# jianfch/stable-ts

Measured on AMD Instinct MI355X. Metric: real-time factor (audio-sec/wall-sec) large-v3 word_timestamps=True, higher is better.
Workload: dtype f16; 1 GPU; large-v3 (random-init, weight recipe BENCH_WEIGHTS = the parity-pinned recipe of tests/test_gpu_f16_depth.py), 10 min synthetic 16 kHz audio per GPU, word_timestamps=True, beam_size=5, 112 decode steps/window, window-parallel batch 20, default regrouping inside the timed pass; mode=transcribe, windows_per_gpu=20, segments=125, words=1670, parallelism=dp1 (windows sharded, no data-path collective)

## Files before the change

stable_ts_amd/csrc/swx_decode.hip:

```cpp
#include "swx_common.h"
#include "swx_kernels.h"
#include "swx_decode.h"

namespace {

constexpr int SEL_T = 1024;
constexpr float NEG_INF = -__builtin_inff();

struct ArgMax { float v; int i; };

__device__ __forceinline__ ArgMax argmax_combine(ArgMax a, ArgMax b)
{
    if (b.v > a.v || (b.v == a.v && b.i < a.i)) return b;
    return a;
}

static_assert(SEL_T == 1024, "block reductions: 16 wave slots");

__device__ ArgMax block_argmax(ArgMax x, ArgMax *sh)
{
    const int wave = threadIdx.x >> 6, lane = threadIdx.x & 63;
#define SWX_ARGMAX_STEP(O) { ArgMax y; y.v = lane_xor<O>(x.v, lane); y.i = lane_xor<O>(x.i, lane); x = argmax_combine(x, y); }
    SWX_ARGMAX_STEP(32) SWX_ARGMAX_STEP(16) SWX_ARGMAX_STEP(8) SWX_ARGMAX_STEP(4) SWX_ARGMAX_STEP(2) SWX_ARGMAX_STEP(1)
    __syncthreads();
    if (lane == 0) sh[wave] = x;
    __syncthreads();
#ifdef SWX_SELECT_R5_REDUCE
    ArgMax r = sh[0];
    for (int w = 1; w < (int)(blockDim.x >> 6); ++w) r = argmax_combine(r, sh[w]);
    return r;
#else
    x = sh[lane & 15];
    SWX_ARGMAX_STEP(8) SWX_ARGMAX_STEP(4) SWX_ARGMAX_STEP(2) SWX_ARGMAX_STEP(1)
    return x;
#endif
#undef SWX_ARGMAX_STEP
}

__device__ float block_max(float x, float *sh)
{
    x = wave_max(x);
    const int wave = threadIdx.x >> 6, lane = threadIdx.x & 63;
    __syncthreads();
    if (lane == 0) sh[wave] = x;
    __syncthreads();
#if defined(SWX_SELECT_R5_REDUCE) || defined(SWX_SELECT_MAX_WALK)
    float r = sh[0];
    for (int w = 1; w < (int)(blockDim.x >> 6); ++w) r = fmaxf(r, sh[w]);
    return r;
#else
    const f32x4 *s4 = (const f32x4 *)sh;
    float r = -__builtin_inff();
#pragma unroll
    for (int q = 0; q < 4; ++q) { const f32x4 v = s4[q]; r = fmaxf(r, fmaxf(fmaxf(v[0], v[1]), fmaxf(v[2], v[3]))); }
    return r;
#endif
}

__device__ float block_sum(float x, float *sh)
{
    x = wave_sum(x);
    const int wave = threadIdx.x >> 6, lane = threadIdx.x & 63;
    __syncthreads();
    if (lane == 0) sh[wave] = x;
    __syncthreads();
    float r = 0.f;
#if defined(SWX_SELECT_R5_REDUCE) || defined(SWX_SELECT_SUM_WALK)
    for (int w = 0; w < (int)(blockDim.x >> 6); ++w) r += sh[w];
#else
    const f32x4 *s4 = (const f32x4 *)sh;
#pragma unroll
    for (int q = 0; q < 4; ++q) { const f32x4 v = s4[q]; r += v[0]; r += v[1]; r += v[2]; r += v[3]; }
#endif
    return r;
}

__device__ __forceinline__ unsigned hash32(unsigned x)
{
    x ^= x >> 16; x *= 0x7feb352du; x ^= x >> 15; x *= 0x846ca68bu; x ^= x >> 16;
    return x;
}

__device__ __forceinline__ float gumbel(uint64_t seed, unsigned row_uid, unsigned step, unsigned idx)
{
    unsigned h = hash32((unsigned)seed ^ hash32(idx + 0x9e3779b9u * (step + 1u)));
    h = hash32(h ^ hash32(row_uid * 0x85ebca6bu + (unsigned)(seed >> 32)));
    const float u = ((float)(h >> 8) + 0.5f) * (1.0f / 16777216.0f);
    return -logf(-logf(u));
}

__device__ __forceinline__ int win_begin(const DecodeBufs &b, int w) { return b.begin ? b.begin[w] : b.n_init; }

__global__ void decode_init_kernel(DecodeBufs b, const int32_t *__restrict__ init_tokens)
{
    const int r = blockIdx.x;
    const int w = r / b.G;
    const int n0 = win_begin(b, w);
    int32_t *row0 = b.tokens[0] + (size_t)r * b.TS;
    int32_t *row1 = b.tokens[1] + (size_t)r * b.TS;
    for (int i = threadIdx.x; i < b.TS; i += blockDim.x) {
        const int32_t t = (i < n0) ? init_tokens[(size_t)w * b.n_init + i] : b.cfg.eot;
        row0[i] = t;
        row1[i] = t;
    }
    if (threadIdx.x == 0) {
        b.pos0[r] = 0;
        b.sum_lp[r] = 0.f;
        b.row_done[r] = 0;
        if (r % b.G == 0) { b.win_done[w] = 0; b.fin_count[w] = 0; }
        if (r == 0) { *b.n_done = 0; *b.step_dev = 0; }
    }
}

__global__ void decode_after_prefill_kernel(DecodeBufs b)
{
    const int r = blockIdx.x;
    const int w = r / b.G;
    const int n0 = win_begin(b, w);
    if (b.anc[0]) {
        for (int p = threadIdx.x; p < b.n_ctx; p += blockDim.x) {
            const int v = (p < n0) ? w * b.G : r;
            b.anc[0][(size_t)r * b.n_ctx + p] = v;
            b.anc[1][(size_t)r * b.n_ctx + p] = v;
        }
    }
    if (threadIdx.x == 0) b.pos0[r] = n0 - 1;
}

__global__ __launch_bounds__(SEL_T) void decode_prefill_logits_kernel(DecodeBufs b, const float *__restrict__ lg2,
                                                                      float *__restrict__ nospeech)
{
    __shared__ __attribute__((aligned(16))) float sh[SEL_T / 64];
    const int r = blockIdx.x, w = r / b.G, V = b.V;
    const float *last = lg2 + ((size_t)w * 2 + 1) * V;
    float *dst = b.logits + (size_t)r * V;
    for (int i = threadIdx.x; i < V; i += SEL_T) dst[i] = last[i];
    if (r % b.G == 0 && nospeech) {
        const float *sot = lg2 + ((size_t)w * 2) * V;
        float mx = NEG_INF;
        for (int i = threadIdx.x; i < V; i += SEL_T) mx = fmaxf(mx, sot[i]);
        mx = block_max(mx, sh);
        float sum = 0.f;
        for (int i = threadIdx.x; i < V; i += SEL_T) sum += expf(sot[i] - mx);
        sum = block_sum(sum, sh);
        if (threadIdx.x == 0) nospeech[w] = (b.cfg.no_speech >= 0) ? expf(sot[b.cfg.no_speech] - mx) / sum : NAN;
    }
}

__global__ __launch_bounds__(SEL_T) void decode_select_kernel(DecodeBufs b, int cur)
{
    const int step = *b.step_dev;
    __shared__ __attribute__((aligned(16))) float shf[SEL_T / 64];
    __shared__ __attribute__((aligned(16))) ArgMax sha[SEL_T / 64];
    __shared__ int sh_last_ts;
    const int r = blockIdx.x, w = r / b.G, V = b.V, tid = threadIdx.x;
    const swx_decode_cfg &c = b.cfg;
    if (b.win_done[w]) return;
    float *lg = b.logits + (size_t)r * V;
    int32_t *tok = b.tokens[cur] + (size_t)r * b.TS;
    const int n0 = win_begin(b, w);
    const int len = n0 + step;
    const int nsamp = step;
    const int tsb = c.timestamp_begin;

    if (c.suppress_blank && nsamp == 0 && tid == 0) { if (c.blank_token >= 0) lg[c.blank_token] = NEG_INF; lg[c.eot] = NEG_INF; }
    for (int i = tid; i < c.n_suppress; i += SEL_T) { const int t = b.suppress[i]; if ((unsigned)t < (unsigned)V) lg[t] = NEG_INF; }
    if (c.min_tokens > 0 && nsamp < c.min_tokens && tid == 0) lg[c.eot] = NEG_INF;
    __syncthreads();

    if (c.apply_timestamp_rules) {
        if (tid == 0) { sh_last_ts = -1; if (c.no_timestamps >= 0) lg[c.no_timestamps] = NEG_INF; }
        __syncthreads();
        int my = -1;
        for (int i = n0 + tid; i < len; i += SEL_T) if (tok[i] >= tsb) my = i;
        if (my >= 0) atomicMax(&sh_last_ts, my);
        __syncthreads();
        const int last_ts_pos = sh_last_ts;
        const bool last_was_ts = nsamp >= 1 && tok[len - 1] >= tsb;
        const bool penult_was_ts = nsamp < 2 || tok[len - 2] >= tsb;
        int lo0 = 0, hi0 = 0;
        if (last_was_ts) { if (penult_was_ts) { lo0 = tsb; hi0 = V; } else { lo0 = 0; hi0 = c.eot; } }
        int hi1 = tsb;
        if (last_ts_pos >= 0) {
            const int tl = tok[last_ts_pos];
            hi1 = (last_was_ts && !penult_was_ts) ? tl : tl + 1;
        }
        int hi2 = 0;
        int lo3 = V;
        if (nsamp == 0) { hi2 = tsb; if (c.max_initial_timestamp_index >= 0) lo3 = tsb + c.max_initial_timestamp_index + 1; }
        float mx_text = NEG_INF, mx_ts = NEG_INF;
        for (int i = tid; i < V; i += SEL_T) {
            float v = lg[i];
            if ((i >= lo0 && i < hi0) || (i >= tsb && i < hi1) || (i < hi2) || (i >= lo3)) { v = NEG_INF; lg[i] = v; }
            if (i < tsb) mx_text = fmaxf(mx_text, v != v ? -NEG_INF : v); else mx_ts = fmaxf(mx_ts, v);
        }
        mx_text = block_max(mx_text, shf);
        mx_ts = block_max(mx_ts, shf);
        float s_ts = 0.f;
        if (mx_ts > NEG_INF)
            for (int i = tsb + tid; i < V; i += SEL_T) s_ts += expf(lg[i] - mx_ts);
        s_ts = block_sum(s_ts, shf);
        const float lse_ts = (mx_ts > NEG_INF) ? mx_ts + logf(s_ts) : NEG_INF;
        if (lse_ts > mx_text)
            for (int i = tid; i < tsb; i += SEL_T) lg[i] = NEG_INF;
        __syncthreads();
    }

    const uint8_t *tmask = b.ts_mask ? b.ts_mask + (size_t)w * 1501 : nullptr;
    float mx = NEG_INF;
    for (int i = tid; i < V; i += SEL_T) {
        float v = lg[i];
        if (tmask && i >= tsb && i - tsb < 1501 && tmask[i - tsb]) v = NEG_INF;
        if (v != v) v = NEG_INF;
        else if (v == NEG_INF) v = -3.4028234663852886e38f;
        else if (v == -NEG_INF) v = 3.4028234663852886e38f;
        lg[i] = v;
        mx = fmaxf(mx, v);
    }
    mx = block_max(mx, shf);
    float se = 0.f;
    for (int i = tid; i < V; i += SEL_T) se += expf(lg[i] - mx);
    se = block_sum(se, shf);
    const float lse = logf(se);

    if (!c.beam) {
        ArgMax best; best.v = NEG_INF; best.i = 0x7fffffff;
        if (c.temperature == 0.f) {
            for (int i = tid; i < V; i += SEL_T) { ArgMax x; x.v = lg[i]; x.i = i; best = argmax_combine(best, x); }
        } else {
            const float invT = 1.0f / c.temperature;
            const unsigned row_uid = b.win_uid ? (unsigned)b.win_uid[r / b.G] * 0x9E3779B1u + (unsigned)(r % b.G) : (unsigned)r;
            const float *qn = c.noise ? c.noise + ((size_t)step * b.M + r) * V : nullptr;
            for (int i = tid; i < V; i += SEL_T) {
                ArgMax x; x.v = lg[i] * invT + (qn ? -logf(qn[i]) : gumbel(c.seed, row_uid, (unsigned)step, (unsigned)i)); x.i = i;
                best = argmax_combine(best, x);
            }
        }
        best = block_argmax(best, sha);
        if (tid == 0) {
            int next = best.i;
            const bool prev_eot = tok[len - 1] == c.eot;
            const float lp = (lg[next] - mx) - lse;
            if (!prev_eot) b.sum_lp[r] += lp; else next = c.eot;
            tok[len] = next;
            if (len < b.n_ctx) b.pos0[r] = len;
            b.row_done[r] = (next == c.eot) ? 1 : 0;
        }
    } else {
        const int K = b.G + 1;
        for (int k = 0; k < K; ++k) {
            ArgMax best; best.v = NEG_INF; best.i = 0x7fffffff;
            for (int i = tid; i < V; i += SEL_T) { ArgMax x; x.v = lg[i]; x.i = i; best = argmax_combine(best, x); }
            best = block_argmax(best, sha);
            if (tid == 0) {
                b.cand_lp[(size_t)r * K + k] = (best.v - mx) - lse;
                b.cand_tok[(size_t)r * K + k] = best.i;
                lg[best.i] = NEG_INF;
            }
            __syncthreads();
        }
    }
}

template <int NV>
__global__ __launch_bounds__(SEL_T) void decode_select_reg_kernel(DecodeBufs b, int cur)
{
    const int step = *b.step_dev;
    __shared__ __attribute__((aligned(16))) float shf[SEL_T / 64];
    __shared__ __attribute__((aligned(16))) ArgMax sha[SEL_T / 64];
    __shared__ float sh_rot[SEL_T];
    __shared__ int sh_last_ts;
    __shared__ float sh_raw;
    const int r = blockIdx.x, w = r / b.G, V = b.V, tid = threadIdx.x;
    const swx_decode_cfg &c = b.cfg;
    if (b.win_done[w]) return;
    float *lg = b.logits + (size_t)r * V;
    int32_t *tok = b.tokens[cur] + (size_t)r * b.TS;
    const int n0 = win_begin(b, w);
    const int len = n0 + step;
    const int nsamp = step;
    const int tsb = c.timestamp_begin;

    if (c.suppress_blank && nsamp == 0 && tid == 0) { if (c.blank_token >= 0) lg[c.blank_token] = NEG_INF; lg[c.eot] = NEG_INF; }
    for (int i = tid; i < c.n_suppress; i += SEL_T) { const int t = b.suppress[i]; if ((unsigned)t < (unsigned)V) lg[t] = NEG_INF; }
    if (c.min_tokens > 0 && nsamp < c.min_tokens && tid == 0) lg[c.eot] = NEG_INF;
    if (c.apply_timestamp_rules && tid == 0) { sh_last_ts = -1; if (c.no_timestamps >= 0) lg[c.no_timestamps] = NEG_INF; }
    __syncthreads();

    float v[NV];
#pragma unroll
    for (int k = 0; k < NV; ++k) { const int i = tid + k * SEL_T; v[k] = i < V ? lg[i] : NEG_INF; }

    if (c.apply_timestamp_rules) {
        int my = -1;
        for (int i = n0 + tid; i < len; i += SEL_T) if (tok[i] >= tsb) my = i;
        if (my >= 0) atomicMax(&sh_last_ts, my);
        __syncthreads();
        const int last_ts_pos = sh_last_ts;
        const bool last_was_ts = nsamp >= 1 && tok[len - 1] >= tsb;
        const bool penult_was_ts = nsamp < 2 || tok[len - 2] >= tsb;
        int lo0 = 0, hi0 = 0;
        if (last_was_ts) { if (penult_was_ts) { lo0 = tsb; hi0 = V; } else { lo0 = 0; hi0 = c.eot; } }
        int hi1 = tsb;
        if (last_ts_pos >= 0) {
            const int tl = tok[last_ts_pos];
            hi1 = (last_was_ts && !penult_was_ts) ? tl : tl + 1;
        }
        int hi2 = 0, lo3 = V;
        if (nsamp == 0) { hi2 = tsb; if (c.max_initial_timestamp_index >= 0) lo3 = tsb + c.max_initial_timestamp_index + 1; }
        float mx_text = NEG_INF, mx_ts = NEG_INF;
#pragma unroll
        for (int k = 0; k < NV; ++k) {
            const int i = tid + k * SEL_T;
            if (i < V) {
                if ((i >= lo0 && i < hi0) || (i >= tsb && i < hi1) || (i < hi2) || (i >= lo3)) v[k] = NEG_INF;
                if (i < tsb) mx_text = fmaxf(mx_text, v[k] != v[k] ? -NEG_INF : v[k]); else mx_ts = fmaxf(mx_ts, v[k]);
            }
        }
        mx_text = block_max(mx_text, shf);
        mx_ts = block_max(mx_ts, shf);
        float s_own = 0.f;
        if (mx_ts > NEG_INF) {
#pragma unroll
            for (int k = 0; k < NV; ++k) { const int i = tid + k * SEL_T; if (i >= tsb && i < V) s_own += expf(v[k] - mx_ts); }
        }
        sh_rot[(tid - tsb) & (SEL_T - 1)] = s_own;
        __syncthreads();
        float s_ts = block_sum(sh_rot[tid], shf);
        const float lse_ts = (mx_ts > NEG_INF) ? mx_ts + logf(s_ts) : NEG_INF;
        if (lse_ts > mx_text) {
#pragma unroll
            for (int k = 0; k < NV; ++k) if (tid + k * SEL_T < tsb) v[k] = NEG_INF;
        }
    }

    const uint8_t *tmask = b.ts_mask ? b.ts_mask + (size_t)w * 1501 : nullptr;
    float mx = NEG_INF;
#pragma unroll
    for (int k = 0; k < NV; ++k) {
        const int i = tid + k * SEL_T;
        if (i < V) {
            float x = v[k];
            if (tmask && i >= tsb && i - tsb < 1501 && tmask[i - tsb]) x = NEG_INF;
            if (x != x) x = NEG_INF;
            else if (x == NEG_INF) x = -3.4028234663852886e38f;
            else if (x == -NEG_INF) x = 3.4028234663852886e38f;
            v[k] = x;
            mx = fmaxf(mx, x);
        }
    }
    mx = block_max(mx, shf);
    float se = 0.f;
#pragma unroll
    for (int k = 0; k < NV; ++k) if (tid + k * SEL_T < V) se += expf(v[k] - mx);
    se = block_sum(se, shf);
    const float lse = logf(se);

    if (!c.beam) {
        ArgMax best; best.v = NEG_INF; best.i = 0x7fffffff;
        float raw_own = 0.f;
        if (c.temperature == 0.f) {
#pragma unroll
            for (int k = 0; k < NV; ++k) {
                const int i = tid + k * SEL_T;
                if (i < V) { ArgMax x; x.v = v[k]; x.i = i; const ArgMax nb = argmax_combine(best, x); if (nb.i != best.i) raw_own = v[k]; best = nb; }
            }
        } else {
            const float invT = 1.0f / c.temperature;
            const unsigned row_uid = b.win_uid ? (unsigned)b.win_uid[r / b.G] * 0x9E3779B1u + (unsigned)(r % b.G) : (unsigned)r;
            const float *qn = c.noise ? c.noise + ((size_t)step * b.M + r) * V : nullptr;
#pragma unroll
            for (int k = 0; k < NV; ++k) {
                const int i = tid + k * SEL_T;
                if (i < V) {
                    ArgMax x; x.v = v[k] * invT + (qn ? -logf(qn[i]) : gumbel(c.seed, row_uid, (unsigned)step, (unsigned)i)); x.i = i;
                    const ArgMax nb = argmax_combine(best, x);
                    if (nb.i != best.i) raw_own = v[k];
                    best = nb;
                }
            }
        }
        const int own_i = best.i;
        best = block_argmax(best, sha);
        if (own_i == best.i) sh_raw = raw_own;
        __syncthreads();
        if (tid == 0) {
            int next = best.i;
            const bool prev_eot = tok[len - 1] == c.eot;
            const float lp = (sh_raw - mx) - lse;
            if (!prev_eot) b.sum_lp[r] += lp; else next = c.eot;
            tok[len] = next;
            if (len < b.n_ctx) b.pos0[r] = len;
            b.row_done[r] = (next == c.eot) ? 1 : 0;
        }
    } else {
        const int K = b.G + 1;
        auto local_best = [&]() {
            ArgMax best; best.v = NEG_INF; best.i = 0x7fffffff;
#pragma unroll
            for (int k = 0; k < NV; ++k) {
                const int i = tid + k * SEL_T;
                if (i < V) { ArgMax x; x.v = v[k]; x.i = i; best = argmax_combine(best, x); }
            }
            return best;
        };
        ArgMax mine = local_best();
        for (int kk = 0; kk < K; ++kk) {
            const ArgMax best = block_argmax(mine, sha);
            if (tid == 0) {
                b.cand_lp[(size_t)r * K + kk] = (best.v - mx) - lse;
                b.cand_tok[(size_t)r * K + kk] = best.i;
            }
            if ((best.i & (SEL_T - 1)) == tid) {
#pragma unroll
                for (int k = 0; k < NV; ++k) if (tid + k * SEL_T == best.i) v[k] = NEG_INF;
                mine = local_best();
            }
        }
    }
}

__global__ __launch_bounds__(256) void decode_beam_update_kernel(DecodeBufs b, int cur)
{
    const int step = *b.step_dev;
    constexpr int MAXC = 17 * 16;
    __shared__ float sc[MAXC];
    __shared__ short src[MAXC];
    __shared__ int tk[MAXC];
    __shared__ short order[MAXC];
    __shared__ int sel_src[16], sel_tok[16];
    __shared__ float sel_sc[16];
    const int w = blockIdx.x, G = b.G, K = G + 1, tid = threadIdx.x;
    const swx_decode_cfg &c = b.cfg;
    __shared__ int s_frozen;
    if (tid == 0) s_frozen = b.win_done[w];
    __syncthreads();
    const bool frozen = s_frozen != 0;
    const int len = win_begin(b, w) + step;
    const int nb = (step == 0) ? 1 : G;
    const int nc = nb * K;
    if (!frozen) {
        for (int ci = tid; ci < nc; ci += 256) {
            const int j = ci / K, k = ci - j * K, idx = w * G + j;
            sc[ci] = b.sum_lp[idx] + b.cand_lp[(size_t)idx * K + k];
            src[ci] = (short)idx;
            tk[ci] = b.cand_tok[(size_t)idx * K + k];
        }
    }
    __syncthreads();
    if (!frozen) {
        for (int ci = tid; ci < nc; ci += 256) {
            const float raw = sc[ci], mine = (raw != raw) ? -INFINITY : raw;
            int rank = 0;
            for (int q = 0; q < nc; ++q) {
                const float rq = sc[q], oq = (rq != rq) ? -INFINITY : rq;
                rank += (oq > mine || (oq == mine && q < ci)) ? 1 : 0;
            }
            order[rank] = (short)ci;
        }
    }
    __syncthreads();
    if (frozen) {
        if (tid < G) sel_src[tid] = w * G + tid;
    } else if (tid == 0) {
        int saved = 0;
        int fc = b.fin_count[w];
        for (int a = 0; a < nc && saved < G; ++a) {
            const int ci = order[a];
            if (tk[ci] == c.eot) {
                if (fc < b.max_cand) {
                    int32_t *ft = b.fin_tokens + ((size_t)w * b.fin_cap + fc) * b.TS;
                    const int32_t *st = b.tokens[cur] + (size_t)src[ci] * b.TS;
                    for (int i = 0; i < len; ++i) ft[i] = st[i];
                    for (int i = len; i < b.TS; ++i) ft[i] = c.eot;
                    b.fin_score[(size_t)w * b.fin_cap + fc] = sc[ci];
                    b.fin_len[(size_t)w * b.fin_cap + fc] = len + 1;
                    ++fc;
                }
            } else {
                sel_src[saved] = src[ci]; sel_tok[saved] = tk[ci]; sel_sc[saved] = sc[ci];
                ++saved;
            }
        }
        b.fin_count[w] = fc;
        if (fc >= b.max_cand) b.win_done[w] = 1;
    }
    __syncthreads();
    for (int s = 0; s < G; ++s) {
        const int dst = w * G + s, from = sel_src[s];
        const int32_t *st = b.tokens[cur] + (size_t)from * b.TS;
        int32_t *dt = b.tokens[cur ^ 1] + (size_t)dst * b.TS;
        const int32_t *sa = b.anc[cur] + (size_t)from * b.n_ctx;
        int32_t *da = b.anc[cur ^ 1] + (size_t)dst * b.n_ctx;
        if (frozen) {
            for (int i = tid; i < b.TS; i += 256) dt[i] = st[i];
            for (int p = tid; p < b.n_ctx; p += 256) da[p] = sa[p];
        } else {
            for (int i = tid; i < b.TS; i += 256) dt[i] = (i < len) ? st[i] : (i == len ? sel_tok[s] : c.eot);
            for (int p = tid; p < b.n_ctx; p += 256) da[p] = (p < len) ? sa[p] : dst;
            if (tid == 0) { b.sum_lp[dst] = sel_sc[s]; if (len < b.n_ctx) b.pos0[dst] = len; }
        }
    }
}

__global__ __launch_bounds__(64) void decode_step_finish_kernel(DecodeBufs b)
{
    if (blockIdx.x != 0) return;
    const int lane = threadIdx.x;
    const int step = *b.step_dev;
    int nd = 0;
    for (int w = lane; w < b.W; w += 64) {
        int done = b.win_done[w];
        if (!b.cfg.beam && !done) {
            int all = 1;
            for (int g = 0; g < b.G; ++g) all &= b.row_done[w * b.G + g];
            if (all) { b.win_done[w] = 1; done = 1; }
        }
        if (b.begin && !done && b.begin[w] + step + 1 > b.n_ctx) { b.win_done[w] = 1; done = 1; }
        b.win_done_prev[w] = done;
        nd += done ? 1 : 0;
    }
    nd += lane_xor<32>(nd, lane); nd += lane_xor<16>(nd, lane); nd += lane_xor<8>(nd, lane);
    nd += lane_xor<4>(nd, lane); nd += lane_xor<2>(nd, lane); nd += lane_xor<1>(nd, lane);
    if (lane == 0) { *b.n_done = nd; *b.step_dev = step + 1; }
}

__global__ void decode_finalize_kernel(DecodeBufs b, int cur, int n_steps, int32_t *__restrict__ tokens_out,
                                       int32_t *__restrict__ lens_out, float *__restrict__ sumlp_out, int G_out)
{
    const int w = blockIdx.x, tid = threadIdx.x, TS = b.TS;
    const swx_decode_cfg &c = b.cfg;
    __shared__ int n_out;
    __shared__ int pick[16];
    if (!c.beam) {
        for (int g = 0; g < b.G; ++g) {
            const int32_t *st = b.tokens[cur] + (size_t)(w * b.G + g) * TS;
            int32_t *dt = tokens_out + ((size_t)w * G_out + g) * TS;
            for (int i = tid; i < TS; i += blockDim.x) dt[i] = st[i];
            if (tid == 0) sumlp_out[(size_t)w * G_out + g] = b.sum_lp[w * b.G + g];
        }
        if (tid == 0) n_out = b.G;
    } else {
        if (tid == 0) {
            int fc = b.fin_count[w];
            int np = 0;
            if (fc < b.G) {
                bool used[16];
                for (int g = 0; g < b.G; ++g) used[g] = false;
                while (fc + np < b.G) {
                    int bj = -1;
                    for (int g = b.G - 1; g >= 0; --g)
                        if (!used[g] && (bj < 0 || b.sum_lp[w * b.G + g] > b.sum_lp[w * b.G + bj])) bj = g;
                    used[bj] = true;
                    pick[np++] = bj;
                }
            }
            n_out = fc + np;
        }
        __syncthreads();
        const int fc = b.fin_count[w];
        for (int k = 0; k < n_out; ++k) {
            int32_t *dt = tokens_out + ((size_t)w * G_out + k) * TS;
            if (k < fc) {
                const int32_t *st = b.fin_tokens + ((size_t)w * b.fin_cap + k) * TS;
                for (int i = tid; i < TS; i += blockDim.x) dt[i] = st[i];
                if (tid == 0) sumlp_out[(size_t)w * G_out + k] = b.fin_score[(size_t)w * b.fin_cap + k];
            } else {
                const int g = pick[k - fc];
                const int32_t *st = b.tokens[cur] + (size_t)(w * b.G + g) * TS;
                for (int i = tid; i < TS; i += blockDim.x) dt[i] = st[i];
                if (tid == 0) sumlp_out[(size_t)w * G_out + k] = b.sum_lp[w * b.G + g];
            }
        }
    }
    __syncthreads();
    for (int k = tid; k < G_out; k += blockDim.x) {
        if (k >= n_out) { lens_out[(size_t)w * G_out + k] = -1; continue; }
    }
    __syncthreads();
    if (tid == 0) {
        for (int k = 0; k < n_out; ++k) {
            const int32_t *dt = tokens_out + ((size_t)w * G_out + k) * TS;
            const int n0 = win_begin(b, w);
            int e = n0;
            while (e < TS && dt[e] != c.eot) ++e;
            lens_out[(size_t)w * G_out + k] = e - n0;
        }
    }
}

}

int swx_decode_init(const DecodeBufs &b, const int32_t *init_tokens, hipStream_t s)
{
    hipLaunchKernelGGL(decode_init_kernel, dim3(b.M), dim3(256), 0, s, b, init_tokens);
    SWX_CHECK_LAUNCH();
    return 0;
}
int swx_decode_after_prefill(const DecodeBufs &b, const float *lg2, float *nospeech, hipStream_t s)
{
    hipLaunchKernelGGL(decode_after_prefill_kernel, dim3(b.M), dim3(256), 0, s, b);
    hipLaunchKernelGGL(decode_prefill_logits_kernel, dim3(b.M), dim3(SEL_T), 0, s, b, lg2, nospeech);
    SWX_CHECK_LAUNCH();
    return 0;
}
int swx_decode_select(const DecodeBufs &b, int cur, hipStream_t s)
{
    SwxProfScope prof(PC_SELECT, (double)b.M * b.V * 4.0, s);
    const bool mem_kernel = swx_flags() & SWX_FLAG_SELECT_MEM;
    if (!mem_kernel && b.V <= 51 * SEL_T)
        hipLaunchKernelGGL(decode_select_reg_kernel<51>, dim3(b.M), dim3(SEL_T), 0, s, b, cur);
    else
        hipLaunchKernelGGL(decode_select_kernel, dim3(b.M), dim3(SEL_T), 0, s, b, cur);
    if (b.cfg.beam) {
        hipLaunchKernelGGL(decode_beam_update_kernel, dim3(b.W), dim3(256), 0, s, b, cur);
    }
    hipLaunchKernelGGL(decode_step_finish_kernel, dim3(1), dim3(64), 0, s, b);
    SWX_CHECK_LAUNCH();
    return 0;
}
int swx_decode_finalize(const DecodeBufs &b, int cur, int n_steps, int32_t *tokens_out, int32_t *lens_out,
                        float *sumlp_out, int G_out, hipStream_t s)
{
    hipLaunchKernelGGL(decode_finalize_kernel, dim3(b.W), dim3(256), 0, s, b, cur, n_steps, tokens_out, lens_out, sumlp_out, G_out);
    SWX_CHECK_LAUNCH();
    return 0;
}
```

stable_ts_amd/csrc/swx_kernels.h:

```cpp
#pragma once
#include <hip/hip_runtime.h>
#include <stdint.h>
#include "../../include/swx.h"

#define EPI_BIAS 1
#define EPI_GELU 2
#define EPI_RES 4
#define EPI_OUT_F32 8
#define EPI_RESF32MOD 16
#define EPI_CBATCH 64
#define EPI_STORE_VT 32
#define EPI_KV 128

#define EPI_QKV_VT 256

struct GemmArgs {
    const void *A; int64_t lda;
    const void *W; int64_t ldw;
    const float *bias;
    const void *R; int64_t ldr;
    const float *Rf; int res_mod;
    void *C; int64_t ldc;
    void *C2;
    void *P; int64_t p_bs;
    int p_nkpad, p_vcol0;
    int M, N, K;
    int epi;
    int vt_s, vt_kp; int64_t vt_bs;
    int vt_zero_pad;
    int tile_order;
};
int swx_gemm(int dtype, const GemmArgs &g, int force_kernel, hipStream_t s);
enum { SWX_GEMM_TILED_REG = 0, SWX_GEMM_SKINNY = 1, SWX_GEMM_GLDS128 = 2, SWX_GEMM_GLDS64 = 3, SWX_GEMM_RING64 = 4, SWX_GEMM_RING128 = 5,
       SWX_GEMM_BIG = 6 };
int swx_gemm_plan_f16(int M, int N, int K, int epi, int64_t ldc, int64_t ldr, bool ptr16, int force_kernel, int flags);

#define SWX_FLAG_TABLE(X) \
    X(NO_FAST_STEP, 0)         \
    X(KCACHE_CHUNKED, 1)       \
    X(SELFATTN_NO_DEEP, 2)     \
    X(DEC_NO_W1, 4)            \
    X(TALL_NO_W8, 5)           \
    X(FLASH_NO_QB1, 6)         \
    X(XKV_PACK_SEPARATE, 7)    \
    X(SELFATTN_NO_MQ, 8)       \
    X(XQ_FULL_TILE, 9)         \
    X(DEC_W1_FULL_TILE, 10)    \
    X(NO_PACKED_XKV, 11)       \
    X(SELECT_MEM, 13)          \
    X(NO_GRAPH, 14)            \
    X(NO_PREFETCH, 15)         \
    X(NO_RING, 16)             \
    X(NO_BIG_TILE, 17)         \
    X(SCORE_TILED, 18)         \
    X(NO_TALL, 19)             \
    X(NO_FUSED_XQ, 20)         \
    X(TICKET, 21)              \
    X(BIG8_GROUPED, 22)        \
    X(XKV_TWO_LAUNCHES, 23)    \
    X(LOUDNESS_ONE_WG, 24)     \
    X(XATTN_R5, 25)            \
    X(FLASH_PIPELINED, 26)     \
    X(SELFATTN_WG5, 27)        \
    X(QKV_SEPARATE_VT, 28)
#define SWX_FLAG_DEFINE(name, bit) constexpr int SWX_FLAG_##name = 1 << (bit);
SWX_FLAG_TABLE(SWX_FLAG_DEFINE)
#undef SWX_FLAG_DEFINE
#define SWX_FLAG_IN_RANGE(name, bit) && (bit) >= 0 && (bit) <= 30
#define SWX_FLAG_OR(name, bit) | (int64_t(1) << (bit))
#define SWX_FLAG_SUM(name, bit) + (int64_t(1) << (bit))
static_assert(true SWX_FLAG_TABLE(SWX_FLAG_IN_RANGE), "SWX_FLAG_TABLE: a bit index outside 0..30");
static_assert((int64_t(0) SWX_FLAG_TABLE(SWX_FLAG_OR)) == (int64_t(0) SWX_FLAG_TABLE(SWX_FLAG_SUM)), "SWX_FLAG_TABLE: two switches share a bit");
#undef SWX_FLAG_IN_RANGE
#undef SWX_FLAG_OR
#undef SWX_FLAG_SUM
#define SWX_DEFAULT_FLAGS 0
int swx_flags();

struct KLayout { int sp, sh, sc; };
__host__ __device__ inline KLayout swx_klayout(int chunked, int n_ctx, int d)
{
    return chunked ? KLayout{8, 64 * n_ctx, 8 * n_ctx} : KLayout{d, 64, 8};
}
__host__ __device__ inline int swx_kidx(const KLayout &L, int pos, int h, int chunk) { return h * L.sh + chunk * L.sc + pos * L.sp; }

#define DEC_LN 1
#define DEC_GELU 2
#define DEC_RES 4
#define DEC_QKV 8
#define DEC_SLAB 16
#define DEC_TICKET 32
struct DecPrefetch {
    const void *base;
    int lines;
};
DecPrefetch swx_dec_prefetch_of(const void *packed_w, int M, int N, int K, int epi);

struct DecGemmArgs {
    const _Float16 *A; int64_t lda;
    const _Float16 *W; int64_t ldw;
    int M, N, K;
    int epi;
    const float *c2;
    const float *c1;
    _Float16 *C; int64_t ldc;
    _Float16 *X; int64_t ldx;
    float *slabs;
    int *ticket;
    _Float16 *kcache, *vcache; const int32_t *pos0; int n_ctx, d;
    KLayout kl;
    int rps;
    int row_mul;
    int ks2, kslice, n_rg; int64_t slab_stride;
    int tall;
    int tps;
    DecPrefetch pf;
    int w1_full_tile;
};
#define SWX_DEC_TICKETS 4096
int swx_dec_plan(int M, int N, int K, int epi, int *mt, int *ks2);
size_t swx_dec_slab_floats(int M, int N, int K);
int swx_gemm_dec(DecGemmArgs g, hipStream_t s);
enum SwxDecKernel { SWX_DEC_K_W4 = 0,
                    SWX_DEC_K_W1 = 1,
                    SWX_DEC_K_TALL4 = 2,
                    SWX_DEC_K_TALL8 = 3 };
int swx_dec_kernel_plan(int M, int N, int K, int epi, int tall, bool ticket_ok, int flags, int *mt, int *ks2, bool *ticket);
int swx_fold_ln(const void *W, const float *gamma, const float *beta, const float *bias, void *Wf, float *c1, float *c2,
                int N, int K, hipStream_t s);

enum SwxProfClass { PC_GEMM_TILED = 0, PC_GEMM_SKINNY = 1, PC_ATTN_FLASH = 2, PC_ATTN_ROWWISE = 3, PC_SELF_ATTN = 4,
                    PC_SELECT = 5, PC_MEL = 6, PC_ALIGN = 7, PC_DTW = 8, PC_NORM = 9, PC_COUNT = 10 };
bool swx_prof_on();
void swx_prof_begin(int cls, double work, hipStream_t s);
void swx_prof_end(hipStream_t s);
struct SwxProfScope {
    hipStream_t s; bool on;
    SwxProfScope(int cls, double work, hipStream_t st) : s(st), on(swx_prof_on()) { if (on) swx_prof_begin(cls, work, st); }
    ~SwxProfScope() { if (on) swx_prof_end(s); }
};

int swx_layernorm(int dtype, const void *x, int64_t ldx, const float *gamma, const float *beta, void *y, int64_t ldy,
                  int rows, int d, hipStream_t s);
int swx_mel_transpose(int dtype, const float *mel, int B, int n_mels, int Cp, void *melT, hipStream_t s);
int swx_fill_zero(void *p, size_t bytes, hipStream_t s);
int swx_embed(int dtype, const int32_t *tokens, int64_t ld_tok, const int32_t *tok_off, const int32_t *pos0, int R, int n_new,
              const void *tok_emb, const float *pos_emb, int d, void *x, hipStream_t s);
int swx_convert_f32(int dtype, const float *src, void *dst, int64_t n, hipStream_t s);
int swx_copy_rows(int dtype, const float *src, int64_t src_ld, void *dst, int64_t dst_ld, int64_t rows, int64_t cols,
                  hipStream_t s);
int swx_copy_conv_w(int dtype, const float *src, int out_c, int in_c, int in_cp, void *dst, hipStream_t s);

struct AttnArgs {
    const void *q; int64_t ldq;
    const void *k; const void *v; int64_t ldkv;
    int64_t k_bs, v_bs;
    int vt_kp;
    void *o; int64_t ldo;
    int B, H, nq, nk;
    int q_rows_per_batch;
    const void *kv_packed;
    const _Float16 *fq_x; int64_t fq_ldx; int fq_rows;
    const _Float16 *fq_w; const float *fq_c1, *fq_c2; int fq_k;
    const void *fq_pf; int fq_pf_lines;
    int fq_full_tile;
    int f32_no_split;
};
__host__ __device__ inline int64_t swx_xkv_packed_elems_per_head(int nk) { return (int64_t)((nk + 31) / 32) * 4 * 512 * 2; }
int swx_xkv_pack(const void *k, const void *vt, void *packed, int B, int H, int nk, int ldk, int vt_kp, int64_t batch_stride,
                 hipStream_t s);
#define SWX_VT_KP 1536
int swx_attention(int dtype, const AttnArgs &a, int force_kernel, hipStream_t s);
enum SwxXattnFamily { SWX_XA_NOT_DECODE = 0,
                      SWX_XA_ROW = 1,
                      SWX_XA_PACKED = 2,
                      SWX_XA_PACKED_FQ = 3 };
struct SwxXattnPlan { int family, qg, depth; };
SwxXattnPlan swx_xattn_plan(int dtype, const AttnArgs &a, int force_kernel, int flags);
int swx_transpose_v(const void *v, int64_t ldv, int64_t v_bs, int n, void *vt, int kp, int64_t vt_bs, int B, int H, hipStream_t s);
int swx_pad_zero(void *base, int64_t row_bytes, int64_t batch_bytes, int off_bytes, int pad_bytes, int rows, int nb, hipStream_t s);
struct SelfAttnArgs {
    const void *qkv; int64_t ldqkv;
    void *kcache; void *vcache;
    int32_t *anc;
    const int32_t *pos0;
    void *o; int64_t ldo;
    int R, n_new, H, n_ctx, d;
    int skip_append;
    int step_cached;
    int step_pos;
    int pos_bound;
    int pos0_all_zero;
    KLayout kl;
};
int swx_self_attention(int dtype, const SelfAttnArgs &a, int row_mul, hipStream_t s);
enum SwxSelfAttnKernel { SWX_SA_K_CACHED_F16 = 0,
                         SWX_SA_K_CACHED_F32 = 1,
                         SWX_SA_K_MQ4 = 2,
                         SWX_SA_K_MQ8 = 3,
                         SWX_SA_K_STEP = 4,
                         SWX_SA_K_STEP_WG5 = 5,
                         SWX_SA_K_STEP_LONG = 6,
                         SWX_SA_K_STEP_LONG_WG5 = 7,
                         SWX_SA_K_STEP_DEEP = 8 };
int swx_self_attn_plan(int dtype, const SelfAttnArgs &a, int row_mul, int flags);
int swx_qk_capture(int dtype, const void *q, int64_t ldq, int q_rows_per_w, int row0, int n_rows, const void *k,
                   int64_t ldk, int64_t k_bs, int nk, const int32_t *heads, int n_heads, int head_slot0, int slots_total, int W,
                   float *out, int out_ld_n, int out_ld_f, hipStream_t s);

int swx_align_weights_launch(const float *d_qk, float *d_p, float *d_mean, float *d_sd, int W, int H, int N, int ld_f,
                             const int *d_n_rows, const int *d_n_frames, float qk_scale, int medfilt_width,
                             float *d_neg_matrix, int out_ld_n, int out_ld_f, hipStream_t s);
int swx_mel_launch(const float *d_pcm, int B, const float *d_hann, const double2 *d_twiddle, const float *d_filters,
                   int n_mels, float *d_mel, unsigned *d_gmax, int per_item_max, hipStream_t s);
int swx_mel_ragged_launch(const float *d_pcm, const int *d_lens, int B, const float *d_hann, const double2 *d_twiddle,
                          const float *d_filters, int n_mels, float *d_mel, unsigned *d_gmax, int group,
                          hipStream_t s);

constexpr int SWX_HS_MAXF = 1536;
int swx_headsel_dynamic_launch(int dtype, const void *qcap, int max_n, int d, int row0, int n_rows, const void *xkv,
                               int64_t layer_stride, int L, int H, int F, int nk, float qk_scale, int count, const double *d_peaks,
                               double *d_score, int32_t *d_sel, float *d_out, int out_ld_f, hipStream_t s);
int swx_headsel_new_launch(int dtype, const void *qcap, int max_n, int d, int n, int row0, int n_out, const void *xkv,
                           int64_t layer_stride, int L, int H, int F, float qk_scale, int medfilt_width, int topk, float w_col,
                           float w_row, float w_cov, float *d_colnorm, float *d_score, int32_t *d_top, float *d_out, int out_ld_f,
                           hipStream_t s);
int swx_headsel_dynamic_batch_launch(int dtype, const void *qcap, int W, int max_n, int d, int row0, const int32_t *d_n_rows,
                                     int n_rows1, int row_ld, const void *xkv, int64_t layer_stride, int64_t win_stride, int L, int H,
                                     const int32_t *d_n_frames, int F1, int nk, float qk_scale, int count, const double *d_peaks,
                                     double *d_score, int32_t *d_sel, float *d_out, int out_ld_f, hipStream_t s);
int swx_headsel_new_batch_launch(int dtype, const void *qcap, int W, int max_n, int d, const int32_t *d_n_tok, int n1, int row0,
                                 const int32_t *d_n_out, int n_out1, int max_out, const void *xkv, int64_t layer_stride,
                                 int64_t win_stride, int L, int H, const int32_t *d_n_frames, int F1, float qk_scale, int medfilt_width,
                                 int topk, float w_col, float w_row, float w_cov, float *d_colnorm, float *d_score, int32_t *d_top,
                                 float *d_out, int out_ld_n, int out_ld_f, hipStream_t s);
int swx_weighted_sum_launch(const float *const *h_xs, const float *h_coef, int n_in, float *d_out, int64_t n, hipStream_t s);

struct DecodeState;
```

Measured before the change: 1444 x real time.

## Rewrite register-resident decode select kernel with fewer barriers and bitmask suppression

Adds a new templated select kernel (specialised on beam and timestamp-rule flags) that issues the logits loads before any barrier and applies token suppression through a per-thread 64-bit bitmask built in shared memory with atomics. The last-timestamp search now uses one atomicMax, and block reductions read the 16 wave slots with vector loads. The beam top-K loop does a double-buffered wave argmax, so each candidate costs one barrier. The old kernel is kept behind a new flag for parity, at the cost of much more complex code and a risk of subtle masking-rule differences.

```diff
diff --git a/stable_ts_amd/csrc/swx_decode.hip b/stable_ts_amd/csrc/swx_decode.hip
--- a/stable_ts_amd/csrc/swx_decode.hip
+++ b/stable_ts_amd/csrc/swx_decode.hip
@@ -263,7 +263,7 @@
 }
 
 template <int NV>
-__global__ __launch_bounds__(SEL_T) void decode_select_reg_kernel(DecodeBufs b, int cur)
+__global__ __launch_bounds__(SEL_T) void decode_select_reg_parent_kernel(DecodeBufs b, int cur)
 {
     const int step = *b.step_dev;
     __shared__ __attribute__((aligned(16))) float shf[SEL_T / 64];
@@ -407,6 +407,246 @@
         ArgMax mine = local_best();
         for (int kk = 0; kk < K; ++kk) {
             const ArgMax best = block_argmax(mine, sha);
+            if (tid == 0) {
+                b.cand_lp[(size_t)r * K + kk] = (best.v - mx) - lse;
+                b.cand_tok[(size_t)r * K + kk] = best.i;
+            }
+            if ((best.i & (SEL_T - 1)) == tid) {
+#pragma unroll
+                for (int k = 0; k < NV; ++k) if (tid + k * SEL_T == best.i) v[k] = NEG_INF;
+                mine = local_best();
+            }
+        }
+    }
+}
+
+__device__ __forceinline__ float slots16_max(const float *sh)
+{
+    const f32x4 *s4 = (const f32x4 *)sh;
+    float r = -__builtin_inff();
+#pragma unroll
+    for (int q = 0; q < 4; ++q) { const f32x4 v = s4[q]; r = fmaxf(r, fmaxf(fmaxf(v[0], v[1]), fmaxf(v[2], v[3]))); }
+    return r;
+}
+__device__ __forceinline__ float slots16_sum(const float *sh)
+{
+    const f32x4 *s4 = (const f32x4 *)sh;
+    float r = 0.f;
+#pragma unroll
+    for (int q = 0; q < 4; ++q) { const f32x4 v = s4[q]; r += v[0]; r += v[1]; r += v[2]; r += v[3]; }
+    return r;
+}
+#define SWX_ARGMAX_STEP(O) { ArgMax y; y.v = lane_xor<O>(x.v, lane); y.i = lane_xor<O>(x.i, lane); x = argmax_combine(x, y); }
+__device__ __forceinline__ ArgMax wave_argmax(ArgMax x, int lane)
+{
+    SWX_ARGMAX_STEP(32) SWX_ARGMAX_STEP(16) SWX_ARGMAX_STEP(8) SWX_ARGMAX_STEP(4) SWX_ARGMAX_STEP(2) SWX_ARGMAX_STEP(1)
+    return x;
+}
+__device__ __forceinline__ ArgMax slots16_argmax(const ArgMax *sh, int lane)
+{
+    ArgMax x = sh[lane & 15];
+    SWX_ARGMAX_STEP(8) SWX_ARGMAX_STEP(4) SWX_ARGMAX_STEP(2) SWX_ARGMAX_STEP(1)
+    return x;
+}
+#undef SWX_ARGMAX_STEP
+
+template <int NV, bool BEAM, bool RULES>
+__global__ __launch_bounds__(SEL_T) void decode_select_reg_kernel(DecodeBufs b, int cur)
+{
+    static_assert(NV <= 64, "one suppression bit per (thread, k) in two 32-bit words");
+    __shared__ __attribute__((aligned(16))) float sh_mx2[2 * (SEL_T / 64)];
+    __shared__ __attribute__((aligned(16))) float sh_sts[SEL_T / 64];
+    __shared__ __attribute__((aligned(16))) float sh_mx[SEL_T / 64];
+    __shared__ __attribute__((aligned(16))) float sh_se[SEL_T / 64];
+    __shared__ __attribute__((aligned(16))) ArgMax sha[2][SEL_T / 64];
+    __shared__ float sh_rot[SEL_T];
+    __shared__ unsigned sh_sup[2][SEL_T];
+    __shared__ unsigned long long sh_last;
+    __shared__ float sh_raw;
+    const int r = blockIdx.x, w = r / b.G, V = b.V, tid = threadIdx.x;
+    const int lane = tid & 63, wave = __builtin_amdgcn_readfirstlane(tid >> 6);
+    const swx_decode_cfg &c = b.cfg;
+    const int tsb = c.timestamp_begin;
+    const float *lg = b.logits + (size_t)r * V;
+    const int k_full = V / SEL_T, n_last = V % SEL_T;
+    auto valid = [&](int k) { return k < k_full || (k == k_full && tid < n_last); };
+
+    const int step = *b.step_dev;
+    const int frozen = b.win_done[w];
+    const int n0_ragged = *(b.begin ? b.begin + w : b.step_dev);
+    const int n0 = b.begin ? n0_ragged : b.n_init;
+    const int n_sup = c.n_suppress;
+    const int32_t *supp = n_sup > 0 ? b.suppress : (const int32_t *)lg;
+    const int sup0 = supp[tid < n_sup ? tid : (n_sup > 0 ? n_sup - 1 : 0)];
+    const int k1 = tsb > tid ? (tsb - tid + SEL_T - 1) / SEL_T : 0;
+    const int j1 = tid + k1 * SEL_T - tsb;
+    const bool two_ts = j1 + SEL_T < 1501;
+    const uint8_t *tmask = b.ts_mask ? b.ts_mask + (size_t)w * 1501 : (const uint8_t *)lg;
+    const int m1 = tmask[b.ts_mask ? j1 : 0];
+    const int m2 = tmask[b.ts_mask && two_ts ? j1 + SEL_T : 0];
+    const int len = n0 + step;
+    const int nsamp = step;
+    int32_t *tok = b.tokens[cur] + (size_t)r * b.TS;
+    auto tok_at = [&](int i) { return tok[i < 0 ? 0 : (i < b.TS ? i : b.TS - 1)]; };
+    const int t_last = tok_at(len - 1), t_penult = tok_at(len - 2);
+    int my_tok = tok_at(n0 + tid);
+    float v[NV];
+#pragma unroll
+    for (int k = 0; k < NV; ++k) { const int i = tid + k * SEL_T; v[k] = lg[i < V ? i : V - 1]; }
+
+    sh_sup[0][tid] = 0u; sh_sup[1][tid] = 0u;
+    if (tid == 0) sh_last = 0ull;
+    __syncthreads();
+    if (frozen) return;
+    if (tid < n_sup && (unsigned)sup0 < (unsigned)V) atomicOr(&sh_sup[(sup0 >> 15) & 1][sup0 & (SEL_T - 1)], 1u << ((sup0 >> 10) & 31));
+    for (int i = tid + SEL_T; i < n_sup; i += SEL_T) {
+        const int t = b.suppress[i];
+        if ((unsigned)t < (unsigned)V) atomicOr(&sh_sup[(t >> 15) & 1][t & (SEL_T - 1)], 1u << ((t >> 10) & 31));
+    }
+    int my = -1;
+    if constexpr (RULES) {
+        if (n0 + tid < len && my_tok >= tsb) my = n0 + tid;
+        for (int i = n0 + tid + SEL_T; i < len; i += SEL_T) { const int t = tok[i]; if (t >= tsb) { my = i; my_tok = t; } }
+    }
+    if (my >= 0) atomicMax(&sh_last, ((unsigned long long)(unsigned)(my + 1) << 32) | (unsigned)my_tok);
+    __syncthreads();
+    {
+        const int kv = tid < V ? (V - tid + SEL_T - 1) / SEL_T : 0;
+        unsigned long long sup = kv < 64 ? ~0ull << kv : 0ull;
+        sup |= (unsigned long long)sh_sup[0][tid] | ((unsigned long long)sh_sup[1][tid] << 32);
+        auto strike = [&](int t) { if ((t & (SEL_T - 1)) == tid) sup |= 1ull << ((t >> 10) & 63); };
+        if (c.suppress_blank && nsamp == 0) { if (c.blank_token >= 0) strike(c.blank_token); strike(c.eot); }
+        if (c.min_tokens > 0 && nsamp < c.min_tokens) strike(c.eot);
+        if (RULES && c.no_timestamps >= 0) strike(c.no_timestamps);
+#pragma unroll
+        for (int k = 0; k < NV; ++k) if ((sup >> k) & 1ull) v[k] = NEG_INF;
+    }
+    static_assert(NV + 1 < 64, "k1 + 1 is a shift count of a 64-bit mask");
+    const unsigned tsp = (unsigned)k1 | (b.ts_mask && m1 != 0 ? 0x100u : 0u) | (b.ts_mask && m2 != 0 && two_ts ? 0x200u : 0u);
+
+    bool kill_text = false;
+    if constexpr (RULES) {
+        const unsigned long long lt = sh_last;
+        const int last_ts_pos = __builtin_amdgcn_readfirstlane((int)(unsigned)(lt >> 32)) - 1;
+        const bool last_was_ts = nsamp >= 1 && __builtin_amdgcn_readfirstlane(t_last) >= tsb;
+        const bool penult_was_ts = nsamp < 2 || __builtin_amdgcn_readfirstlane(t_penult) >= tsb;
+        int lo0 = 0, hi0 = 0;
+        if (last_was_ts) { if (penult_was_ts) { lo0 = tsb; hi0 = V; } else { lo0 = 0; hi0 = c.eot; } }
+        int hi1 = tsb;
+        if (last_ts_pos >= 0) {
+            const int tl = __builtin_amdgcn_readfirstlane((int)(unsigned)lt);
+            hi1 = (last_was_ts && !penult_was_ts) ? tl : tl + 1;
+        }
+        int hi2 = 0, lo3 = V;
+        if (nsamp == 0) { hi2 = tsb; if (c.max_initial_timestamp_index >= 0) lo3 = tsb + c.max_initial_timestamp_index + 1; }
+        float mx_text = NEG_INF, mx_ts = NEG_INF;
+#pragma unroll
+        for (int k = 0; k < NV; ++k) {
+            const int i = tid + k * SEL_T;
+            if (valid(k)) {
+                if ((i >= lo0 && i < hi0) || (i >= tsb && i < hi1) || (i < hi2) || (i >= lo3)) v[k] = NEG_INF;
+                if (i < tsb) mx_text = fmaxf(mx_text, v[k] != v[k] ? -NEG_INF : v[k]); else mx_ts = fmaxf(mx_ts, v[k]);
+            }
+        }
+        mx_text = wave_max(mx_text);
+        mx_ts = wave_max(mx_ts);
+        if (lane == 0) { sh_mx2[wave] = mx_text; sh_mx2[SEL_T / 64 + wave] = mx_ts; }
+        __syncthreads();
+        mx_text = slots16_max(sh_mx2);
+        mx_ts = slots16_max(sh_mx2 + SEL_T / 64);
+        float s_own = 0.f;
+        if (mx_ts > NEG_INF) {
+#pragma unroll
+            for (int k = 0; k < NV; ++k) { const int i = tid + k * SEL_T; if (i >= tsb && valid(k)) s_own += expf(v[k] - mx_ts); }
+        }
+        sh_rot[(tid - tsb) & (SEL_T - 1)] = s_own;
+        __syncthreads();
+        float s_ts = wave_sum(sh_rot[tid]);
+        if (lane == 0) sh_sts[wave] = s_ts;
+        __syncthreads();
+        s_ts = slots16_sum(sh_sts);
+        const float lse_ts = (mx_ts > NEG_INF) ? mx_ts + logf(s_ts) : NEG_INF;
+        kill_text = lse_ts > mx_text;
+    }
+
+    const unsigned long long tsm = ((unsigned long long)((tsp >> 8) & 1u) << (tsp & 63u)) | ((unsigned long long)((tsp >> 9) & 1u) << ((tsp & 63u) + 1u));
+    float mx = NEG_INF;
+#pragma unroll
+    for (int k = 0; k < NV; ++k) {
+        if (valid(k)) {
+            float x = v[k];
+            if (kill_text && tid + k * SEL_T < tsb) x = NEG_INF;
+            if ((tsm >> k) & 1ull) x = NEG_INF;
+            if (x != x) x = NEG_INF;
+            else if (x == NEG_INF) x = -3.4028234663852886e38f;
+            else if (x == -NEG_INF) x = 3.4028234663852886e38f;
+            v[k] = x;
+            mx = fmaxf(mx, x);
+        }
+    }
+    mx = wave_max(mx);
+    if (lane == 0) sh_mx[wave] = mx;
+    __syncthreads();
+    mx = slots16_max(sh_mx);
+    float se = 0.f;
+#pragma unroll
+    for (int k = 0; k < NV; ++k) if (valid(k)) se += expf(v[k] - mx);
+    se = wave_sum(se);
+
+    if constexpr (!BEAM) {
+        if (lane == 0) sh_se[wave] = se;
+        __syncthreads();
+        se = slots16_sum(sh_se);
+        const float lse = logf(se);
+        float bv = NEG_INF, raw_own = 0.f;
+        int bk = -1;
+        auto take = [&](int k, float xv) { if (xv > bv || (bk < 0 && xv == bv)) { bv = xv; bk = k; raw_own = v[k]; } };
+        if (c.temperature == 0.f) {
+#pragma unroll
+            for (int k = 0; k < NV; ++k) if (valid(k)) take(k, v[k]);
+        } else {
+            const float invT = 1.0f / c.temperature;
+            const unsigned row_uid = b.win_uid ? (unsigned)b.win_uid[r / b.G] * 0x9E3779B1u + (unsigned)(r % b.G) : (unsigned)r;
+            const float *qn = c.noise ? c.noise + ((size_t)step * b.M + r) * V : nullptr;
+#pragma unroll
+            for (int k = 0; k < NV; ++k) {
+                const int i = tid + k * SEL_T;
+                if (valid(k)) take(k, v[k] * invT + (qn ? -logf(qn[i]) : gumbel(c.seed, row_uid, (unsigned)step, (unsigned)i)));
+            }
+        }
+        ArgMax best; best.v = bv; best.i = bk < 0 ? 0x7fffffff : tid + bk * SEL_T;
+        const int own_i = best.i;
+        best = block_argmax(best, sha[0]);
+        if (own_i == best.i) sh_raw = raw_own;
+        __syncthreads();
+        if (tid == 0) {
+            int next = best.i;
+            const bool prev_eot = t_last == c.eot;
+            const float lp = (sh_raw - mx) - lse;
+            if (!prev_eot) b.sum_lp[r] += lp; else next = c.eot;
+            tok[len] = next;
+            if (len < b.n_ctx) b.pos0[r] = len;
+            b.row_done[r] = (next == c.eot) ? 1 : 0;
+        }
+    } else {
+        const int K = b.G + 1;
+        auto local_best = [&]() {
+            float bv = NEG_INF; int bk = -1;
+            if (tid < V) { bv = v[0]; bk = 0; }
+#pragma unroll
+            for (int k = 1; k < NV; ++k) if (v[k] > bv) { bv = v[k]; bk = k; }
+            ArgMax best; best.v = bv; best.i = bk < 0 ? 0x7fffffff : tid + bk * SEL_T;
+            return best;
+        };
+        ArgMax mine = local_best();
+        if (lane == 0) sh_se[wave] = se;
+        float lse = 0.f;
+        for (int kk = 0; kk < K; ++kk) {
+            const ArgMax wbest = wave_argmax(mine, lane);
+            if (lane == 0) sha[kk & 1][wave] = wbest;
+            __syncthreads();
+            if (kk == 0 && tid == 0) lse = logf(slots16_sum(sh_se));
+            const ArgMax best = slots16_argmax(sha[kk & 1], lane);
             if (tid == 0) {
                 b.cand_lp[(size_t)r * K + kk] = (best.v - mx) - lse;
                 b.cand_tok[(size_t)r * K + kk] = best.i;
@@ -608,8 +848,15 @@
 {
     SwxProfScope prof(PC_SELECT, (double)b.M * b.V * 4.0, s);
     const bool mem_kernel = swx_flags() & SWX_FLAG_SELECT_MEM;
-    if (!mem_kernel && b.V <= 51 * SEL_T)
-        hipLaunchKernelGGL(decode_select_reg_kernel<51>, dim3(b.M), dim3(SEL_T), 0, s, b, cur);
+    const bool reg_parent = swx_flags() & SWX_FLAG_SELECT_REG_PARENT;
+    if (!mem_kernel && b.V <= 51 * SEL_T && reg_parent)
+        hipLaunchKernelGGL(decode_select_reg_parent_kernel<51>, dim3(b.M), dim3(SEL_T), 0, s, b, cur);
+    else if (!mem_kernel && b.V <= 51 * SEL_T) {
+        const bool beam = b.cfg.beam != 0, rules = b.cfg.apply_timestamp_rules != 0;
+        auto kern = beam ? (rules ? decode_select_reg_kernel<51, true, true> : decode_select_reg_kernel<51, true, false>)
+                         : (rules ? decode_select_reg_kernel<51, false, true> : decode_select_reg_kernel<51, false, false>);
+        hipLaunchKernelGGL(kern, dim3(b.M), dim3(SEL_T), 0, s, b, cur);
+    }
     else
         hipLaunchKernelGGL(decode_select_kernel, dim3(b.M), dim3(SEL_T), 0, s, b, cur);
     if (b.cfg.beam) {
diff --git a/stable_ts_amd/csrc/swx_kernels.h b/stable_ts_amd/csrc/swx_kernels.h
--- a/stable_ts_amd/csrc/swx_kernels.h
+++ b/stable_ts_amd/csrc/swx_kernels.h
@@ -39,6 +39,7 @@
     X(NO_FAST_STEP, 0)         \
     X(KCACHE_CHUNKED, 1)       \
     X(SELFATTN_NO_DEEP, 2)     \
+    X(SELECT_REG_PARENT, 3)    \
     X(DEC_NO_W1, 4)            \
     X(TALL_NO_W8, 5)           \
     X(FLASH_NO_QB1, 6)         \
```

Result: no change. 1433 x real time (-0.7%).
